# NVlabs/intrinsic3d

Measured on NVIDIA H100. Metric: gauss_newton_iterations_per_sec, higher is better.
Workload: dtype f32

## Files before the change

intrinsic3d_b200/csrc/i3d_engine.cu:

```cuda
#include <cuda_runtime.h>
#include <dlfcn.h>

#include <algorithm>
#include <chrono>
#include <climits>
#include <cmath>
#include <cstdarg>
#include <cstdio>
#include <cstdlib>
#include <cstring>
#include <string>
#include <vector>

#include "../../include/i3d_c_api.h"
#include "i3d_kernels.cuh"
#include "i3d_lighting.cuh"
#include "i3d_recolor.cuh"
#include "i3d_gridops.cuh"
#include "i3d_host.h"
#include "i3d_frames.h"
#include "i3d_fusion.h"
#include "i3d_mesh.h"
#include "i3d_render.h"
#include "i3d_track.h"
// ... 47 lines not shown
    std::string error;

    int64_t n = 0;
    float voxel_size = 0.f, truncation = 0.f;
    Dev<int32_t> x, y, z, nbr;
    Dev<double> sdf0, sdfA, albA, sdfB, albB, sh;
    Dev<float> weight;
    Dev<uchar4> rgb;
    double* sdf = nullptr; double* alb = nullptr;
    double* c_sdf = nullptr; double* c_alb = nullptr;
    bool have_sh = false;
    int F = 0, W = 0, H = 0;
    double pyr_scale = 1.0;
    Dev<float> lum, depth;
    Dev<float> tile_min, tile_max;
    Dev<unsigned long long> cull_stats;
    Dev<double> camA, camB;
    double* cam = nullptr; double* c_cam = nullptr;
    bool have_cam = false;
    Dev<uint8_t> flags;
    Dev<int32_t> up_xyz, up_vals; Dev<uint8_t> up_rgb; Dev<unsigned long long> up_keys; Dev<int> up_dup; Dev<double> up_sh;
    uint64_t hash_cap = 0;
    Dev<int32_t> sp_x, sp_y, sp_z; Dev<double> sp_sdf0, sp_sdf, sp_alb; Dev<float> sp_w; Dev<uchar4> sp_rgb;
    Dev<int32_t> act, scan_counts, scan_total;
    int n_active = 0, K = 0, stride = 0;
    Dev<float> Rt;
    Dev<FramePose> pose_ctx, pose_ctx_c;
    Dev<int32_t> obs_frame, row_frame;
    Dev<float> obs_w;
    Dev<float4> Jt;
    Dev<float2> Jtail;
    Dev<double> row_res, row_wraw;
    Dev<float> ea_w;
    Dev<double> lap;
    Dev<float> cam_acc;
    Dev<double> minv, type_w;
    Dev<int> fail_flag;
    Dev<float> v_bg, v_cg, v_s, v_jtj, v_b, v_x, v_r, v_z, v_p, v_ps, v_qg, v_tr, v_delta;
    Dev<double> v_bgd, v_cgd, v_qgd, cam_accd;
    Dev<CgCtl> ctl;
    Dev<double> red_partials, red_out;
    Dev<unsigned int> red_counters;
    size_t max_blocks = 0;
    bool keep_raw = false;
    Dev<float> dbg_v;
    I3DParams last_params{};
    bool have_iter = false;
    Timing timing;
    int64_t launches = 0;
    int64_t host_syncs = 0;
    Dev<IterDev> iter_dev;
    int last_cg_iterations = 4, prev_cg_iterations = 4;
    bool pcg_fused = true;
    int64_t step_n = -1;
    unsigned step_grid = 0; int step_K = 0; size_t step_smem = 0;
    Dev<uint8_t> color;
    bool have_color = false;
    Dev<unsigned long long> recolor_counts;
    Dev<int32_t> sv_table, sv_index, sv_nbr;
    Dev<int> sv_scalars, sv_deg;
    Dev<double> sv_acc, sv_work;
    Dev<I3DLightingInfo> sv_info;
    Dev<uint8_t> sh_has;
    int sv_S = 0;
    double* sv_x = nullptr;
    SubvolGrid sv_grid{};
    FusionState fusion;
    ScoreScratch scores;
    RgbdStore rgbd;
    SensorStore sensor;
    MeshState mesh;
    RenderState render;
    TrackScratch track;
    int64_t shard_begin = 0, shard_end = -1;
    int rank = 0, world = 1;
    NcclApi::Comm comm = nullptr;
    bool shard_ready = false;
    Dev<uint8_t> held;
    Dev<uint8_t> held_mask;
    Dev<int32_t> slist;
    int64_t n_shared = 0;
    int64_t hv0 = 0, hv1 = 0;
    int64_t loc_begin = 0, loc_end = 0;
    Dev<double> xbuf;
    Dev<uint8_t> mbox;
    size_t mbox_cap = 0;
    bool p2p_ready = false;
    unsigned int xseq = 0;
    std::vector<void*> peer_base;
    Dev<double*> d_peer_data;
    Dev<unsigned int*> d_peer_flags;
    static constexpr size_t kMboxFlagBytes = 4096;
    P2PView p2p_view() const { P2PView v; v.rank = rank; v.world = world; v.peer_data = d_peer_data.p; v.peer_flags = d_peer_flags.p; v.cap = mbox_cap; return v; }
    Shard shard() const
    {
        Shard sh;
        if (world > 1) { sh.own_begin = shard_begin; sh.own_end = shard_end; sh.hv0 = hv0; sh.hv1 = hv1; sh.cam_owner = (rank == 0); sh.defer = 1; sh.loc_begin = loc_begin; sh.loc_end = loc_end; }
        else { sh.own_begin = 0; sh.own_end = n; sh.hv0 = 0; sh.hv1 = n; sh.cam_owner = 1; sh.defer = 0; sh.loc_begin = 0; sh.loc_end = n; }
        return sh;
    }
    int64_t held_count() const { return (world > 1 ? 2 * (hv1 - hv0) : 2 * n) + 6 * static_cast<int64_t>(F) + 9; }
    ShareView share_view() const { ShareView v; v.n_shared = n_shared; v.slist = slist.p; v.held = held_mask.p; return v; }

    int64_t U() const { return 2 * n + 6 * static_cast<int64_t>(F) + 9; }
    ReduceSite site(int s)
    {
// ... 162 lines not shown
    rows.n_active = e->n_active; rows.K = e->K; rows.stride = e->stride; rows.act = e->act.p; rows.Jt = e->Jt.p; rows.Jtail = e->Jtail.p;
    rows.row_frame = e->row_frame.p; rows.row_res = e->row_res.p; rows.row_wraw = e->row_wraw.p;
    return rows;
}

RegView reg_view(I3DEngine* e, const I3DParams& P)
{
    RegView rv;
    rv.flags = e->flags.p; rv.ea_w = e->ea_w.p; rv.lap = e->lap.p;
    rv.use_er = P.use_er; rv.use_es = P.use_es; rv.use_ea = P.use_ea;
    return rv;
}

SelectCam select_cam(const I3DEngine* e, const double hc9[9], float occlusion)
{
    SelectCam sc;
    sc.fx = static_cast<float>(hc9[0] * e->pyr_scale); sc.fy = static_cast<float>(hc9[1] * e->pyr_scale);
    sc.cx = static_cast<float>(hc9[2] * e->pyr_scale); sc.cy = static_cast<float>(hc9[3] * e->pyr_scale);
    sc.dist_zero = 1;
    for (int k = 0; k < 5; ++k) { sc.d[k] = static_cast<float>(hc9[4 + k]); if (sc.d[k] != 0.0f) sc.dist_zero = 0; }
    sc.occlusion = occlusion;
    return sc;
}

CullView cull_view(const I3DEngine* e, unsigned long long* stats)
{
    static const bool no_cull = std::getenv("I3D_NO_CULL") != nullptr;
    return CullView{e->tile_min.p, e->tile_max.p, no_cull ? 0 : 1, stats};
}

#define NK(call)                                                            \
    do {                                                                    \
        int _r = (call);                                                    \
        if (_r != 0) throw NcclError{_r, __LINE__};                         \
    } while (0)


bool pdl_enabled() { static const bool on = [] { const char* v = std::getenv("I3D_PDL"); return !(v && v[0] == '0'); }(); return on; }

template <bool COOPERATIVE = false, class... KArgs, class... Args>
void pdl_launch(I3DEngine* e, void (*kern)(KArgs...), unsigned grid, unsigned block, size_t smem, Args&&... args)
{
    cudaLaunchConfig_t cfg{};
    cfg.gridDim = dim3(grid); cfg.blockDim = dim3(block); cfg.dynamicSmemBytes = smem; cfg.stream = e->stream;
    cudaLaunchAttribute at[2];
    unsigned na = 0;
    if (COOPERATIVE) { at[na].id = cudaLaunchAttributeCooperative; at[na].val.cooperative = 1; ++na; }
    if (pdl_enabled()) { at[na].id = cudaLaunchAttributeProgrammaticStreamSerialization; at[na].val.programmaticStreamSerializationAllowed = 1; ++na; }
    cfg.attrs = at; cfg.numAttrs = na;
    CK(cudaLaunchKernelEx(&cfg, kern, static_cast<KArgs>(args)...));
    e->launches += 1;
}

template <int MODE>
void launch_eg_rows(I3DEngine* e, const GridView& g, const CamView& cv, const EgRows& rows, const int32_t* obs_frame, const float* obs_w)
{
    if constexpr (MODE == ROWS_COST)
    {
        const size_t smem = rows_smem_bytes(MODE, 256, true, e->F);
        if (2 * (smem + 1024) <= 227u * 1024u)
        {
            auto kern = k_eg_rows<MODE, 256, true>;
            CK(cudaFuncSetAttribute(kern, cudaFuncAttributeMaxDynamicSharedMemorySize, static_cast<int>(smem)));
            pdl_launch(e, kern, blocks_for(static_cast<size_t>(rows.stride), 256), 256, smem, g, e->frame_view(), cv, rows, obs_frame, obs_w, e->site(SITE_EG_COST));
            return;
        }
    }
    auto kern = k_eg_rows<MODE, 128, false>;
    const size_t smem = rows_smem_bytes(MODE, 128, false, e->F);
    CK(cudaFuncSetAttribute(kern, cudaFuncAttributeMaxDynamicSharedMemorySize, static_cast<int>(smem)));
    pdl_launch(e, kern, blocks_for(static_cast<size_t>(rows.stride), 128), 128, smem, g, e->frame_view(), cv, rows, obs_frame, obs_w, e->site(SITE_EG_COST));
}

void allreduce_scalars(I3DEngine* e, double* dev, int count, int kind, int respect_done)
{
    if (e->world <= 1) return;
    if (e->p2p_ready && count <= 30)
    {
        const unsigned int seq = ++e->xseq;
        pdl_launch(e, k_xchg_scalars, 1, 32, 0, e->p2p_view(), seq, dev, count, e->ctl.p, kind, respect_done);
        return;
    }
    NK(g_nccl.AllReduce(dev, dev, static_cast<size_t>(count), NCCL_FLOAT64, NCCL_SUM, e->comm, e->stream));
    if (kind >= 0) pdl_launch(e, k_epilogue, 1, 32, 0, e->ctl.p, dev, kind, respect_done);
}

void exchange(I3DEngine* e, float* v0, float* v1, float* extra_f, int n_extra_f, double* extra_d, int n_extra_d, int respect_done, int epilogue_kind = -1)
{
    if (e->world <= 1) return;
    const ShareView shv = e->share_view();
    const size_t nv = v1 ? 2 : 1;
    const size_t total = nv * static_cast<size_t>(e->n_shared) + n_extra_f + n_extra_d;
    const size_t threads = static_cast<size_t>(e->n_shared) + n_extra_f + n_extra_d;
    if (e->p2p_ready && total <= e->mbox_cap)
    {
        const unsigned int seq = ++e->xseq;
        double* buf = reinterpret_cast<double*>(e->mbox.p + I3DEngine::kMboxFlagBytes) + static_cast<size_t>(seq & 1u) * e->mbox_cap;
        pdl_launch(e, k_pack, blocks_for(threads), kThreads, 0, shv, v0, v1, extra_f, n_extra_f, extra_d, n_extra_d, buf, e->ctl.p, respect_done);
        pdl_launch(e, k_xchg_pull, blocks_for(threads), kThreads, 0, e->p2p_view(), seq, shv, v0, v1, extra_f, n_extra_f, extra_d, n_extra_d, e->ctl.p, respect_done, epilogue_kind);
        return;
    }
    e->xbuf.ensure(2 * static_cast<size_t>(e->n_shared) + CamAccLayout{e->F}.size() + 64);
    pdl_launch(e, k_pack, blocks_for(threads), kThreads, 0, shv, v0, v1, extra_f, n_extra_f, extra_d, n_extra_d, e->xbuf.p, e->ctl.p, respect_done);
    NK(g_nccl.AllReduce(e->xbuf.p, e->xbuf.p, total, NCCL_FLOAT64, NCCL_SUM, e->comm, e->stream));
    pdl_launch(e, k_unpack, blocks_for(threads), kThreads, 0, shv, v0, v1, extra_f, n_extra_f, extra_d, n_extra_d, e->xbuf.p, e->ctl.p, respect_done);
    if (epilogue_kind >= 0) pdl_launch(e, k_epilogue, 1, 32, 0, e->ctl.p, extra_d, epilogue_kind, respect_done);
}

size_t apply_smem_bytes(int F, int K)
{
    return static_cast<size_t>((6 * F + 9 + 15) & ~15) * sizeof(double) + static_cast<size_t>(14 + 6 * K) * kThreads * sizeof(float);
}

size_t accum_smem_bytes(int F, int K)
{
    return static_cast<size_t>((CamAccLayout{F}.size() + 15) & ~15) * sizeof(double) + static_cast<size_t>(K) * 8 * kThreads * sizeof(float);
}

int check_frame_limit(I3DEngine* e, int F, int K)
{
    int optin = 0;
    CK(cudaDeviceGetAttribute(&optin, cudaDevAttrMaxSharedMemoryPerBlockOptin, e->device));
    cudaFuncAttributes fa_acc{}, fa_app{};
    CK(cudaFuncGetAttributes(&fa_acc, k_eg_accum));
// ... 425 lines not shown
    double hc9[9];
    CK(cudaMemcpyAsync(hc9, e->cam + 6 * static_cast<size_t>(F), 9 * sizeof(double), cudaMemcpyDeviceToHost, st));
    CK(cudaStreamSynchronize(st));
    const SelectCam sc = select_cam(e, hc9, 0.0f);
    if (!(std::isfinite(sc.fx) && sc.fx > 0.0f && std::isfinite(sc.fy) && sc.fy > 0.0f && std::isfinite(sc.cx) && std::isfinite(sc.cy)))
        return fail(e, "i3d_render_keyframes: the camera needs finite intrinsics with fx, fy > 0 (fx %g, fy %g, cx %g, cy %g after pyr_scale %g)",
                    sc.fx, sc.fy, sc.cx, sc.cy, e->pyr_scale);
    for (int k = 0; k < 5; ++k)
        if (!std::isfinite(sc.d[k])) return fail(e, "i3d_render_keyframes: distortion coefficient %d is not finite", k);
    RenderCam cam;
    cam.fx = sc.fx; cam.fy = sc.fy; cam.cx = sc.cx; cam.cy = sc.cy; cam.dist_zero = sc.dist_zero;
    for (int k = 0; k < 5; ++k) cam.d[k] = sc.d[k];
    e->render.rt.ensure(12 * static_cast<size_t>(F));
    k_pose_mats<<<blocks_for(F, 64), 64, 0, st>>>(F, e->cam, e->render.rt.p);
    render::keyframes(e->render, e->timing, render_grid(e, P.sdf_source, P.photometric != 0), cam, e->render.rt.p, n, ids, e->W, e->H, e->depth.p,
                      e->lum.p, P.planes, P.photometric != 0, stats, st);
    return 0;
}

}

extern "C" {

int i3d_abi_version(void) { return I3D_ABI_VERSION; }
uint64_t i3d_sizeof_params(void) { return sizeof(I3DParams); }
uint64_t i3d_sizeof_iter_info(void) { return sizeof(I3DIterInfo); }

void i3d_default_params(I3DParams* p)
{
    std::memset(p, 0, sizeof(*p));
    p->lambda[0] = 0.2; p->lambda[1] = 80.0; p->lambda[2] = 120.0; p->lambda[3] = 0.1;
    p->use_er = p->use_es = p->use_ea = 1;
    p->occlusion_distance = 0.02f; p->num_observations = 5; p->lm_steps = 50;
    p->initial_trust_region_radius = 1e4; p->max_trust_region_radius = 1e16; p->min_trust_region_radius = 1e-32;
    p->min_relative_decrease = 1e-3; p->min_lm_diagonal = 1e-6; p->max_lm_diagonal = 1e32; p->eta = 0.1;
    p->function_tolerance = 1e-6; p->gradient_tolerance = 1e-10; p->parameter_tolerance = 1e-8;
    p->max_linear_solver_iterations = 500; p->min_linear_solver_iterations = 0; p->residual_reset_period = 10;
    p->max_consecutive_invalid_steps = 5;
}

int i3d_engine_create(int device, I3DEngine** out)
{
    *out = nullptr;
    int count = 0;
    cudaError_t err = cudaGetDeviceCount(&count);
    if (err != cudaSuccess || count <= 0) return fail(nullptr, "i3d_engine_create: no CUDA device available (%s); this engine has no CPU fallback", cudaGetErrorString(err));
    if (device < 0 || device >= count) return fail(nullptr, "i3d_engine_create: device %d out of range (%d devices)", device, count);
    cudaDeviceProp prop;
    if (cudaGetDeviceProperties(&prop, device) != cudaSuccess) return fail(nullptr, "i3d_engine_create: cannot query device %d", device);
    if (prop.major != 9 || prop.minor != 0) return fail(nullptr, "i3d_engine_create: device %d is sm_%d%d; this library is built for sm_90a (H100) only", device, prop.major, prop.minor);
    I3DEngine* e = new I3DEngine();
    e->device = device;
    { const char* v = std::getenv("I3D_PCG_FUSED"); e->pcg_fused = !(v && v[0] == '0'); }
    const int rc = guarded(e, [&]() {
        CK(cudaStreamCreateWithFlags(&e->stream, cudaStreamNonBlocking));
        e->timing.pool.resize(4096);
        for (auto& ev : e->timing.pool) CK(cudaEventCreate(&ev));
        return 0;
    });
    if (rc != 0) { g_create_error = e->error; delete e; return rc; }
    *out = e;
    return 0;
}

void i3d_engine_destroy(I3DEngine* e)
{
    if (!e) return;
    cudaSetDevice(e->device);
    cudaStreamSynchronize(e->stream);
    for (size_t r = 0; r < e->peer_base.size(); ++r)
        if (static_cast<int>(r) != e->rank && e->peer_base[r]) cudaIpcCloseMemHandle(e->peer_base[r]);
    if (e->comm && g_nccl.CommDestroy) g_nccl.CommDestroy(e->comm);
    for (auto& ev : e->timing.pool) cudaEventDestroy(ev);
    if (e->mesh.ev_ready) for (auto& ev : e->mesh.ev) cudaEventDestroy(ev);
    cudaStreamDestroy(e->stream);
    delete e;
}

const char* i3d_last_error(const I3DEngine* e) { return e ? e->error.c_str() : g_create_error.c_str(); }

int i3d_upload_grid(I3DEngine* e, int64_t n, const int32_t* xyz, const double* sdf0, const double* sdf_refined, const double* albedo,
                    const float* weight, const uint8_t* rgb, float voxel_size)
{
    if (!e) return 1;
    if (n <= 0 || n > (1ll << 30)) return fail(e, "i3d_upload_grid: bad voxel count %lld", static_cast<long long>(n));
    return guarded(e, [&]() {
        cudaStream_t st = e->stream;
        e->n = n; e->voxel_size = voxel_size; e->truncation = voxel_size * 5.0f;
        forget_voxel_set(e);
        e->x.ensure(n); e->y.ensure(n); e->z.ensure(n); e->nbr.ensure(static_cast<size_t>(NB_COUNT) * n);
        e->sdf0.ensure(n); e->sdfA.ensure(n); e->sdfB.ensure(n); e->albA.ensure(n); e->albB.ensure(n); e->weight.ensure(n); e->rgb.ensure(n);
        e->sdf = e->sdfA.p; e->c_sdf = e->sdfB.p; e->alb = e->albA.p; e->c_alb = e->albB.p;
        e->up_xyz.ensure(3 * static_cast<size_t>(n)); e->up_rgb.ensure(3 * static_cast<size_t>(n));
        CK(cudaMemcpyAsync(e->up_xyz.p, xyz, 3 * n * sizeof(int32_t), cudaMemcpyHostToDevice, st));
        CK(cudaMemcpyAsync(e->up_rgb.p, rgb, 3 * n, cudaMemcpyHostToDevice, st));
        CK(cudaMemcpyAsync(e->sdf0.p, sdf0, n * sizeof(double), cudaMemcpyHostToDevice, st));
        CK(cudaMemcpyAsync(e->sdf, sdf_refined, n * sizeof(double), cudaMemcpyHostToDevice, st));
        CK(cudaMemcpyAsync(e->alb, albedo, n * sizeof(double), cudaMemcpyHostToDevice, st));
        CK(cudaMemcpyAsync(e->weight.p, weight, n * sizeof(float), cudaMemcpyHostToDevice, st));
        k_deinterleave_xyz<<<blocks_for(n), kThreads, 0, st>>>(n, e->up_xyz.p, e->x.p, e->y.p, e->z.p, e->up_rgb.p, e->rgb.p);
        const int hdup = rebuild_topology(e);
        if (hdup) return fail(e, "i3d_upload_grid: duplicate voxel coordinates");
        return 0;
    });
}

// ... 1348 lines not shown
```

intrinsic3d_b200/csrc/i3d_kernels.cuh:

```cuda
#pragma once
#include <cuda_runtime.h>
#include <cooperative_groups.h>
#include <stdint.h>
#include <limits.h>
#include "i3d_math.cuh"
#include "i3d_grid.cuh"
#include "i3d_observe.cuh"
#include "../../include/i3d_types.h"

namespace i3d
{

enum : uint8_t { FL_VALID = 1, FL_ACTIVE = 2, FL_RING = 4, FL_FREE_SDF = 8, FL_FREE_ALB = 16, FL_ES_JAC = 32, FL_ROW = 64  };

struct Shard
{
    int64_t own_begin, own_end;
    int64_t hv0, hv1;
    int cam_owner;
    int defer;
    int64_t loc_begin, loc_end;
    __device__ __forceinline__ bool owns_voxel(int64_t v) const { return v >= own_begin && v < own_end; }
    __device__ __forceinline__ bool owns_unknown(int64_t j, int64_t n) const
    {
// ... 480 lines not shown
    for (int k = 0; k < 10; ++k) s10[k] = sdf[idx[k]];
#pragma unroll
    for (int k = 0; k < 4; ++k) a4[k] = alb[idx[10 + k]];
    return true;
}

__device__ __forceinline__ double sdf_to_weight(double sdf, double truncation)
{
    const double a = fmin(fabs(sdf), truncation) / truncation;
    return fmin(fmax(1.0 - a, 0.01), 1.0);
}

struct CamAccLayout
{
    int F;
    __host__ __device__ int pose_stride() const { return 33; }
    __host__ __device__ int tail() const { return 33 * F; }
    __host__ __device__ int size() const { return 33 * F + 43; }
};

enum { ROWS_BUILD = 0, ROWS_COST = 1 };
constexpr int kRowThreads = 128;

__device__ __forceinline__ uint32_t smem_u32(const void* p) { return static_cast<uint32_t>(__cvta_generic_to_shared(p)); }
__device__ __forceinline__ void mbar_init(uint64_t* bar, uint32_t count)
{
    asm volatile("mbarrier.init.shared::cta.b64 [%0], %1;" ::"r"(smem_u32(bar)), "r"(count) : "memory");
    asm volatile("fence.mbarrier_init.release.cluster;" ::: "memory");
}
__device__ __forceinline__ void mbar_expect_tx(uint64_t* bar, uint32_t bytes)
{
    asm volatile("mbarrier.arrive.expect_tx.shared::cta.b64 _, [%0], %1;" ::"r"(smem_u32(bar)), "r"(bytes) : "memory");
}
__device__ __forceinline__ void bulk_copy_g2s(void* dst_smem, const void* src_gmem, uint32_t bytes , uint64_t* bar)
{
    asm volatile("cp.async.bulk.shared::cluster.global.mbarrier::complete_tx::bytes [%0], [%1], %2, [%3];"
                 ::"r"(smem_u32(dst_smem)), "l"(src_gmem), "r"(bytes), "r"(smem_u32(bar)) : "memory");
}
__device__ __forceinline__ void mbar_wait(uint64_t* bar, uint32_t parity)
{
    uint32_t done = 0;
    while (!done)
        asm volatile("{\n\t.reg .pred P1;\n\tmbarrier.try_wait.parity.shared::cta.b64 P1, [%1], %2;\n\tselp.b32 %0, 1, 0, P1;\n\t}"
                     : "=r"(done) : "r"(smem_u32(bar)), "r"(parity) : "memory");
}

static_assert(kVoxelGeomWords == 15, "VoxelGeom size changed: update the pose-table staging boundary and its test");
__host__ __device__ inline size_t rows_pose_bytes(int F) { return (static_cast<size_t>(F) * sizeof(FramePose) + 127) & ~static_cast<size_t>(127); }
__host__ __device__ inline size_t rows_smem_bytes(int mode, int threads, bool stage, int F)
{
    return (stage ? 128 + rows_pose_bytes(F) : 0) + static_cast<size_t>(threads) * (kVoxelGeomWords * sizeof(double) + (mode == ROWS_BUILD ? kVoxelDerivWords * sizeof(float) : 0));
}

template <int MODE, int THREADS, bool STAGE>
__global__ void __launch_bounds__(THREADS, THREADS == 128 ? 4 : 2)
k_eg_rows(GridView g, FrameView fr, CamView cv, EgRows rows, const int32_t* __restrict__ obs_frame, const float* __restrict__ obs_w, ReduceSite site)
{
    extern __shared__ __align__(128) unsigned char s_rows[];
    pdl_prologue();
    uint64_t* s_bar = reinterpret_cast<uint64_t*>(s_rows);
    const FramePose* s_pose = reinterpret_cast<const FramePose*>(s_rows + 128);
    unsigned char* s_state = s_rows + (STAGE ? 128 + rows_pose_bytes(fr.F) : 0);
    double* s_vg = reinterpret_cast<double*>(s_state);
    float* s_vd = reinterpret_cast<float*>(s_state + static_cast<size_t>(THREADS) * kVoxelGeomWords * sizeof(double));
    if (STAGE)
    {
        if (threadIdx.x == 0)
        {
            const uint32_t bytes = static_cast<uint32_t>(fr.F * sizeof(FramePose));
            mbar_init(s_bar, 1);
            mbar_expect_tx(s_bar, bytes);
            bulk_copy_g2s(s_rows + 128, cv.fpose, bytes, s_bar);
        }
        __syncthreads();
    }
    const int a = blockIdx.x * blockDim.x + threadIdx.x;
    double acc[1] = {0.0};
    const VoxelGeomView vg{s_vg + threadIdx.x, THREADS};
    const VoxelDerivView vd{s_vd + threadIdx.x, THREADS};
    bool ok = a < rows.n_active;
    double wsdf = 0.0;
    if (ok)
    {
        const int64_t v = rows.act[a];
        int32_t idx[14];
        double s10[10], a4[4];
        ok = gather_stencil(g, g.sdf, g.albedo, v, idx, s10, a4);
        if (ok)
        {
            double sh[9];
#pragma unroll
            for (int k = 0; k < 9; ++k) sh[k] = g.sh[static_cast<int64_t>(k) * g.n + v];
            const int coord[3] = {g.x[v], g.y[v], g.z[v]};
            VoxelGeom vg_r;
            VoxelDeriv vd_r;
            voxel_geom_make<MODE == ROWS_BUILD>(s10, a4, coord, static_cast<double>(g.voxel_size), sh, &vg_r, &vd_r);
            voxel_geom_park(vg_r, s_vg + threadIdx.x, THREADS);
            if (MODE == ROWS_BUILD) voxel_deriv_park(vd_r, s_vd + threadIdx.x, THREADS);
            if (MODE == ROWS_BUILD) wsdf = sdf_to_weight(s10[0], static_cast<double>(g.truncation));
        }
    }
    if (STAGE) mbar_wait(s_bar, 0);
    if (a < rows.stride)
    {
        CamParams<double> cam;
        make_cam_params(cv, fr.pyr_scale, fr.W, fr.H, &cam);
        const size_t img_stride = static_cast<size_t>(fr.W) * fr.H;
        const int32_t* __restrict__ fsrc = (MODE == ROWS_BUILD) ? obs_frame : rows.row_frame;
        int f_next = ok ? fsrc[a] : -1;
#pragma unroll 1
        for (int k = 0; k < rows.K; ++k)
        {
            const size_t slot = static_cast<size_t>(k) * rows.stride + a;
            const int f = f_next;
            if (ok && k + 1 < rows.K) f_next = fsrc[slot + rows.stride];
            if (!STAGE && f_next >= 0)
            {
                const char* pf = reinterpret_cast<const char*>(cv.fpose + f_next);
                asm volatile("prefetch.global.L1 [%0];" ::"l"(pf));
                asm volatile("prefetch.global.L1 [%0];" ::"l"(pf + 128));
            }
            int32_t rf = -1; double res = 0.0, wraw = 0.0;
            if (f >= 0)
            {
                const FramePose& fp = STAGE ? s_pose[f] : cv.fpose[f];
                PointSave sv[4];
                float e[4];
                res = eg_frame_primal<MODE == ROWS_BUILD>(vg, fp, cam, LinearImage{fr.lum + img_stride * f}, sv, e);
                if (MODE == ROWS_BUILD)
                {
                    if (res != 0.0)
                    {
                        CamParams<float> cf;
                        cf.fx = static_cast<float>(cam.fx); cf.fy = static_cast<float>(cam.fy); cf.cx = static_cast<float>(cam.cx); cf.cy = static_cast<float>(cam.cy);
                        cf.k1 = static_cast<float>(cam.k1); cf.k2 = static_cast<float>(cam.k2); cf.k3 = static_cast<float>(cam.k3);
                        cf.p1 = static_cast<float>(cam.p1); cf.p2 = static_cast<float>(cam.p2);
                        cf.pyr_scale = static_cast<float>(cam.pyr_scale); cf.w = cam.w; cf.h = cam.h;
                        float row[29];
                        eg_frame_deriv(vd, fp, cf, sv, e, row);
                        rf = f;
                        wraw = static_cast<double>(obs_w[slot]) * wsdf;
                        rows.store_row(slot, row);
                    }
                }
                else acc[0] += rows.row_wraw[slot] * res * res;
            }
            if (MODE == ROWS_BUILD) { rows.row_frame[slot] = rf; rows.row_res[slot] = res; rows.row_wraw[slot] = wraw; }
        }
    }
    if (MODE == ROWS_COST) grid_reduce<1>(acc, site);
}

__global__ void __launch_bounds__(kThreads)
k_eg_accum(GridView g, EgRows rows, int F, double* __restrict__ bg, double* __restrict__ cg, double* __restrict__ cam_acc ,
           ReduceSite site )
{
    pdl_prologue();
    extern __shared__ double s_dyn_d[];
    const CamAccLayout lay{F};
    double* s_cam = s_dyn_d;
    float* s_park = reinterpret_cast<float*>(s_dyn_d + ((lay.size() + 15) & ~15));
    for (int i = threadIdx.x; i < lay.size(); i += blockDim.x) s_cam[i] = 0.0;
    __syncthreads();
    const int tid = threadIdx.x, lane = tid & 31;
    const int a = blockIdx.x * blockDim.x + tid;
    const bool in_range = a < rows.n_active;
    double acc[3] = {0.0, 0.0, 0.0};
    float gsum[14], csum[14];
#pragma unroll
    for (int m = 0; m < 14; ++m) { gsum[m] = 0.0f; csum[m] = 0.0f; }
    float tl[64];
#pragma unroll
    for (int i = 0; i < 64; ++i) tl[i] = 0.0f;
    int fk[I3D_MAX_OBS];
#pragma unroll
    for (int k = 0; k < I3D_MAX_OBS; ++k)
    {
        fk[k] = -1;
        if (k >= rows.K) continue;
        const size_t slot = static_cast<size_t>(k) * rows.stride + (in_range ? a : 0);
        const int f = in_range ? rows.row_frame[slot] : -1;
        fk[k] = f;
        if (f >= 0)
        {
            float row[29];
            rows.load_row<false>(slot, row);
            const double wraw = rows.row_wraw[slot], res = rows.row_res[slot];
            const float wf = static_cast<float>(wraw), wr = static_cast<float>(wraw * res);
            acc[0] += wraw; acc[1] += wraw * res * res; acc[2] += 1.0;
#pragma unroll
            for (int m = 0; m < 14; ++m) { gsum[m] += wr * row[m]; csum[m] += wf * row[m] * row[m]; }
#pragma unroll
            for (int m = 0; m < 9; ++m) { tl[m] += wr * row[20 + m]; tl[9 + m] += wf * row[20 + m] * row[20 + m]; }
            int t = 18;
#pragma unroll
            for (int r = 0; r < 4; ++r)
#pragma unroll
                for (int c = r; c < 4; ++c) tl[t++] += wf * row[20 + r] * row[20 + c];
#pragma unroll
            for (int r = 0; r < 5; ++r)
// ... 1507 lines not shown
```

intrinsic3d_b200/csrc/i3d_math.cuh:

```cuda
#pragma once

#ifndef I3D_HD
#ifdef __CUDACC__
#define I3D_HD __host__ __device__ __forceinline__
#else
#define I3D_HD inline
#endif
#endif

#include <math.h>

namespace i3d
{

#define I3D_QUAD(i, j) (((i) == 0) ? (((j) == 0) ? 0 : ((j) == 1) ? 6 : ((j) == 2) ? 1 : 4) \
                      : ((i) == 1) ? (((j) == 0) ? 6 : ((j) == 1) ? 9 : ((j) == 2) ? 7 : 8) \
                      : ((i) == 2) ? (((j) == 0) ? 1 : ((j) == 1) ? 7 : ((j) == 2) ? 2 : 3) \
                                   : (((j) == 0) ? 4 : ((j) == 1) ? 8 : ((j) == 2) ? 3 : 5))

template <class T> struct Num;
template <> struct Num<double>
{
    static I3D_HD double sqrt_(double x) { return sqrt(x); }
    static I3D_HD double floor_(double x) { return floor(x); }
// ... 591 lines not shown


template <bool GRAD>
I3D_HD double bicubic_eval(const BicubicSite& s, const float p[16], float* Lu, float* Lv)
{
    double wu[4], wv[4], du[4], dv[4];
    cr_weights<double>(s.xu, wu);
    cr_weights<double>(s.xv, wv);
    if (GRAD) { cr_dweights<double>(s.xu, du); cr_dweights<double>(s.xv, dv); }
    double L = 0.0, lu = 0.0, lv = 0.0;
#pragma unroll
    for (int i = 0; i < 4; ++i)
    {
        const double p0 = static_cast<double>(p[4 * i]), p1 = static_cast<double>(p[4 * i + 1]), p2 = static_cast<double>(p[4 * i + 2]), p3 = static_cast<double>(p[4 * i + 3]);
        const double ri = fma(wu[0], p0, fma(wu[1], p1, fma(wu[2], p2, wu[3] * p3)));
        L = fma(wv[i], ri, L);
        if (GRAD)
        {
            const double rd = fma(du[0], p0, fma(du[1], p1, fma(du[2], p2, du[3] * p3)));
            lu = fma(wv[i], rd, lu);
            lv = fma(dv[i], ri, lv);
        }
    }
    if (GRAD) { *Lu = static_cast<float>(lu); *Lv = static_cast<float>(lv); }
    return L;
}

struct PointSave { float x, y, iz, Lu, Lv; };

template <bool DERIV, class VG, class IMG>
I3D_HD double eg_frame_primal(const VG& vg, const FramePose& fp, const CamParams<double>& cam, const IMG& img,
                              PointSave sv[4], float e[4])
{
    double u[4], v[4];
    bool inb = true;
#pragma unroll
    for (int i = 0; i < 4; ++i)
    {
        const double X0 = vg.Xv(i, 0), X1 = vg.Xv(i, 1), X2 = vg.Xv(i, 2);
        const double Y0 = fp.R[0] * X0 + fp.R[1] * X1 + fp.R[2] * X2 + fp.t[0];
        const double Y1 = fp.R[3] * X0 + fp.R[4] * X1 + fp.R[5] * X2 + fp.t[1];
        const double Y2 = fp.R[6] * X0 + fp.R[7] * X1 + fp.R[8] * X2 + fp.t[2];
        const double iz = rcp_f64(Y2);
        const double x = Y0 * iz, y = Y1 * iz;
        const double r2 = x * x + y * y, r4 = r2 * r2, r6 = r4 * r2;
        const double dc = 1.0 + cam.k1 * r2 + cam.k2 * r4 + cam.k3 * r6;
        const double xd = x * dc + 2.0 * cam.p1 * x * y + cam.p2 * (r2 + 2.0 * x * x);
        const double yd = y * dc + 2.0 * cam.p2 * xd * y + cam.p1 * (r2 + 2.0 * y * y);
        u[i] = cam.fx * xd + cam.cx; v[i] = cam.fy * yd + cam.cy;
        if (u[i] < 0.0 || u[i] > static_cast<double>(cam.w - 1) || v[i] < 0.0 || v[i] > static_cast<double>(cam.h - 1)) inb = false;
        if (DERIV) { sv[i].x = static_cast<float>(x); sv[i].y = static_cast<float>(y); sv[i].iz = static_cast<float>(iz); }
    }
    double L[4];
#pragma unroll
    for (int i = 0; i < 4; i += 2)
    {
        BicubicSite s0, s1;
        bicubic_locate(u[i], v[i], cam.w, cam.h, &s0);
        bicubic_locate(u[i + 1], v[i + 1], cam.w, cam.h, &s1);
        float p0[16], p1[16];
        img.taps2(cam.w, cam.h, s0, s1, p0, p1);
        float lu = 0.0f, lv = 0.0f;
        L[i] = bicubic_eval<DERIV>(s0, p0, &lu, &lv);
        if (DERIV) { sv[i].Lu = lu; sv[i].Lv = lv; }
        L[i + 1] = bicubic_eval<DERIV>(s1, p1, &lu, &lv);
        if (DERIV) { sv[i + 1].Lu = lu; sv[i + 1].Lv = lv; }
    }
    if (!inb) return 0.0;
    const double d1 = vg.dSv(0) - (L[1] - L[0]);
    const double d2 = vg.dSv(1) - (L[2] - L[0]);
    const double d3 = vg.dSv(2) - (L[3] - L[0]);
    const double r = sqrt(d1 * d1 + d2 * d2 + d3 * d3);
    if (!finite_(r)) return 0.0;
    if (DERIV && r != 0.0)
    {
        const double ir = 1.0 / r;
        e[0] = static_cast<float>(-(d1 + d2 + d3) * ir); e[1] = static_cast<float>(d1 * ir); e[2] = static_cast<float>(d2 * ir); e[3] = static_cast<float>(d3 * ir);
    }
    return r;
}

template <class VD>
I3D_HD void eg_frame_deriv(const VD& vd, const FramePose& fp, const CamParams<float>& cam, const PointSave sv[4], const float e[4],
                           float* __restrict__ row)
{
#pragma unroll
    for (int k = 0; k < 29; ++k) row[k] = 0.0f;
    float m[3] = {0.0f, 0.0f, 0.0f};
    float tacc[3] = {0.0f, 0.0f, 0.0f};
#define I3D_POINT_DERIV(POINT)                                                                                                        \
    {                                                                                                                                 \
        const int i = POINT;                                                                                                          \
        const float x = sv[i].x, y = sv[i].y, iz = sv[i].iz, Lu = sv[i].Lu, Lv = sv[i].Lv, ei = e[i];                                 \
        const float r2 = x * x + y * y, r4 = r2 * r2, r6 = r4 * r2;                                                                   \
        const float dc = 1.0f + cam.k1 * r2 + cam.k2 * r4 + cam.k3 * r6;                                                              \
        const float dcp = cam.k1 + 2.0f * cam.k2 * r2 + 3.0f * cam.k3 * r4;                                                           \
        const float xd = x * dc + 2.0f * cam.p1 * x * y + cam.p2 * (r2 + 2.0f * x * x);                                               \
        const float yd = y * dc + 2.0f * cam.p2 * xd * y + cam.p1 * (r2 + 2.0f * y * y);                                              \
        const float xdx = dc + 2.0f * x * x * dcp + 2.0f * cam.p1 * y + 6.0f * cam.p2 * x;                                            \
        const float xdy = 2.0f * x * y * dcp + 2.0f * cam.p1 * x + 2.0f * cam.p2 * y;                                                 \
        const float ydx = 2.0f * x * y * dcp + 2.0f * cam.p2 * y * xdx + 2.0f * cam.p1 * x;                                           \
        const float ydy = dc + 2.0f * y * y * dcp + 2.0f * cam.p2 * (y * xdy + xd) + 6.0f * cam.p1 * y;                              \
        const float gu = Lu * cam.fx, gv = Lv * cam.fy;                                                                               \
        const float Lx = gu * xdx + gv * ydx, Ly = gu * xdy + gv * ydy;                                                               \
        const float LY0 = Lx * iz, LY1 = Ly * iz, LY2 = -(Lx * x + Ly * y) * iz;                                                      \
        const float LX0 = LY0 * fp.Rf[0] + LY1 * fp.Rf[3] + LY2 * fp.Rf[6];                                                           \
        const float LX1 = LY0 * fp.Rf[1] + LY1 * fp.Rf[4] + LY2 * fp.Rf[7];                                                           \
        const float LX2 = LY0 * fp.Rf[2] + LY1 * fp.Rf[5] + LY2 * fp.Rf[8];                                                           \
        const float s = vd.sv(i), g0 = vd.gv(i, 0), g1 = vd.gv(i, 1), g2 = vd.gv(i, 2);                                              \
        const float Xf0 = vd.X0v(0) + (i == 1 ? vd.hv() : 0.0f) - g0 * s;                                                            \
        const float Xf1 = vd.X0v(1) + (i == 2 ? vd.hv() : 0.0f) - g1 * s;                                                            \
        const float Xf2 = vd.X0v(2) + (i == 3 ? vd.hv() : 0.0f) - g2 * s;                                                            \
        const float c0 = fp.small ? LY0 : LX0, c1 = fp.small ? LY1 : LX1, c2 = fp.small ? LY2 : LX2;                                  \
        m[0] += ei * (Xf1 * c2 - Xf2 * c1); m[1] += ei * (Xf2 * c0 - Xf0 * c2); m[2] += ei * (Xf0 * c1 - Xf1 * c0);                   \
        tacc[0] += ei * LY0; tacc[1] += ei * LY1; tacc[2] += ei * LY2;                                                                \
        row[20] -= ei * (Lu * cam.pyr_scale * xd);                                                                                    \
        row[21] -= ei * (Lv * cam.pyr_scale * yd);                                                                                    \
        row[22] -= ei * (Lu * cam.pyr_scale);                                                                                         \
// ... 36 lines not shown
```

Baseline: 141.2.

## Add optional warp-compacted row evaluation and hoist bicubic site location

Adds a COMPACT variant of the edge-gradient rows kernel. Each warp ballots which (observation, voxel) slots are valid and redistributes the valid work densely across lanes, so lanes with no observation do not sit idle. In cost mode the partial results are shuffled back to the owning lane before the weighted accumulation. The variant only runs when I3D_ROWS_COMPACT=1. Separately, bicubic_locate is computed for all four points before the tap loads, which is always active and may let the loads be issued earlier at the cost of more live registers.

```diff
diff --git a/intrinsic3d_b200/csrc/i3d_engine.cu b/intrinsic3d_b200/csrc/i3d_engine.cu
--- a/intrinsic3d_b200/csrc/i3d_engine.cu
+++ b/intrinsic3d_b200/csrc/i3d_engine.cu
@@ -123,6 +123,7 @@
     Dev<IterDev> iter_dev;
     int last_cg_iterations = 4, prev_cg_iterations = 4;
     bool pcg_fused = true;
+    bool rows_compact = false;
     int64_t step_n = -1;
     unsigned step_grid = 0; int step_K = 0; size_t step_smem = 0;
     Dev<uint8_t> color;
@@ -391,24 +392,30 @@
     e->launches += 1;
 }
 
-template <int MODE>
-void launch_eg_rows(I3DEngine* e, const GridView& g, const CamView& cv, const EgRows& rows, const int32_t* obs_frame, const float* obs_w)
+template <int MODE, bool COMPACT>
+void launch_eg_rows_as(I3DEngine* e, const GridView& g, const CamView& cv, const EgRows& rows, const int32_t* obs_frame, const float* obs_w)
 {
     if constexpr (MODE == ROWS_COST)
     {
         const size_t smem = rows_smem_bytes(MODE, 256, true, e->F);
         if (2 * (smem + 1024) <= 227u * 1024u)
         {
-            auto kern = k_eg_rows<MODE, 256, true>;
+            auto kern = k_eg_rows<MODE, 256, true, COMPACT>;
             CK(cudaFuncSetAttribute(kern, cudaFuncAttributeMaxDynamicSharedMemorySize, static_cast<int>(smem)));
             pdl_launch(e, kern, blocks_for(static_cast<size_t>(rows.stride), 256), 256, smem, g, e->frame_view(), cv, rows, obs_frame, obs_w, e->site(SITE_EG_COST));
             return;
         }
     }
-    auto kern = k_eg_rows<MODE, 128, false>;
+    auto kern = k_eg_rows<MODE, 128, false, COMPACT>;
     const size_t smem = rows_smem_bytes(MODE, 128, false, e->F);
     CK(cudaFuncSetAttribute(kern, cudaFuncAttributeMaxDynamicSharedMemorySize, static_cast<int>(smem)));
     pdl_launch(e, kern, blocks_for(static_cast<size_t>(rows.stride), 128), 128, smem, g, e->frame_view(), cv, rows, obs_frame, obs_w, e->site(SITE_EG_COST));
+}
+template <int MODE>
+void launch_eg_rows(I3DEngine* e, const GridView& g, const CamView& cv, const EgRows& rows, const int32_t* obs_frame, const float* obs_w)
+{
+    if (e->rows_compact) launch_eg_rows_as<MODE, true>(e, g, cv, rows, obs_frame, obs_w);
+    else launch_eg_rows_as<MODE, false>(e, g, cv, rows, obs_frame, obs_w);
 }
 
 void allreduce_scalars(I3DEngine* e, double* dev, int count, int kind, int respect_done)
@@ -940,6 +947,7 @@
     I3DEngine* e = new I3DEngine();
     e->device = device;
     { const char* v = std::getenv("I3D_PCG_FUSED"); e->pcg_fused = !(v && v[0] == '0'); }
+    { const char* v = std::getenv("I3D_ROWS_COMPACT"); e->rows_compact = v && v[0] == '1'; }
     const int rc = guarded(e, [&]() {
         CK(cudaStreamCreateWithFlags(&e->stream, cudaStreamNonBlocking));
         e->timing.pool.resize(4096);
diff --git a/intrinsic3d_b200/csrc/i3d_kernels.cuh b/intrinsic3d_b200/csrc/i3d_kernels.cuh
--- a/intrinsic3d_b200/csrc/i3d_kernels.cuh
+++ b/intrinsic3d_b200/csrc/i3d_kernels.cuh
@@ -556,7 +556,19 @@
     return (stage ? 128 + rows_pose_bytes(F) : 0) + static_cast<size_t>(threads) * (kVoxelGeomWords * sizeof(double) + (mode == ROWS_BUILD ? kVoxelDerivWords * sizeof(float) : 0));
 }
 
-template <int MODE, int THREADS, bool STAGE>
+__device__ __forceinline__ int nth_set_bit(uint32_t m, int n)
+{
+    int pos = 0;
+#pragma unroll
+    for (int w = 16; w > 0; w >>= 1)
+    {
+        const int c = __popc(m & ((1u << w) - 1u));
+        if (n >= c) { n -= c; m >>= w; pos += w; }
+    }
+    return pos;
+}
+
+template <int MODE, int THREADS, bool STAGE, bool COMPACT>
 __global__ void __launch_bounds__(THREADS, THREADS == 128 ? 4 : 2)
 k_eg_rows(GridView g, FrameView fr, CamView cv, EgRows rows, const int32_t* __restrict__ obs_frame, const float* __restrict__ obs_w, ReduceSite site)
 {
@@ -580,8 +592,6 @@
     }
     const int a = blockIdx.x * blockDim.x + threadIdx.x;
     double acc[1] = {0.0};
-    const VoxelGeomView vg{s_vg + threadIdx.x, THREADS};
-    const VoxelDerivView vd{s_vd + threadIdx.x, THREADS};
     bool ok = a < rows.n_active;
     double wsdf = 0.0;
     if (ok)
@@ -605,51 +615,139 @@
         }
     }
     if (STAGE) mbar_wait(s_bar, 0);
-    if (a < rows.stride)
-    {
-        CamParams<double> cam;
-        make_cam_params(cv, fr.pyr_scale, fr.W, fr.H, &cam);
-        const size_t img_stride = static_cast<size_t>(fr.W) * fr.H;
-        const int32_t* __restrict__ fsrc = (MODE == ROWS_BUILD) ? obs_frame : rows.row_frame;
-        int f_next = ok ? fsrc[a] : -1;
+    CamParams<double> cam;
+    make_cam_params(cv, fr.pyr_scale, fr.W, fr.H, &cam);
+    const size_t img_stride = static_cast<size_t>(fr.W) * fr.H;
+    const int32_t* __restrict__ fsrc = (MODE == ROWS_BUILD) ? obs_frame : rows.row_frame;
+    auto row_eval = [&](int col, size_t slot, int f, double wsdf_v, int32_t& rf, double& wraw) -> double {
+        const VoxelGeomView vg{s_vg + col, THREADS};
+        const VoxelDerivView vd{s_vd + col, THREADS};
+        const FramePose& fp = STAGE ? s_pose[f] : cv.fpose[f];
+        PointSave sv[4];
+        float e[4];
+        const double res = eg_frame_primal<MODE == ROWS_BUILD>(vg, fp, cam, LinearImage{fr.lum + img_stride * f}, sv, e);
+        if (MODE == ROWS_BUILD)
+        {
+            if (res != 0.0)
+            {
+                CamParams<float> cf;
+                cf.fx = static_cast<float>(cam.fx); cf.fy = static_cast<float>(cam.fy); cf.cx = static_cast<float>(cam.cx); cf.cy = static_cast<float>(cam.cy);
+                cf.k1 = static_cast<float>(cam.k1); cf.k2 = static_cast<float>(cam.k2); cf.k3 = static_cast<float>(cam.k3);
+                cf.p1 = static_cast<float>(cam.p1); cf.p2 = static_cast<float>(cam.p2);
+                cf.pyr_scale = static_cast<float>(cam.pyr_scale); cf.w = cam.w; cf.h = cam.h;
+                float row[29];
+                eg_frame_deriv(vd, fp, cf, sv, e, row);
+                rf = f;
+                wraw = static_cast<double>(obs_w[slot]) * wsdf_v;
+                rows.store_row(slot, row);
+            }
+        }
+        return res;
+    };
+    if (!COMPACT)
+    {
+        if (a < rows.stride)
+        {
+            int f_next = ok ? fsrc[a] : -1;
 #pragma unroll 1
-        for (int k = 0; k < rows.K; ++k)
-        {
-            const size_t slot = static_cast<size_t>(k) * rows.stride + a;
-            const int f = f_next;
-            if (ok && k + 1 < rows.K) f_next = fsrc[slot + rows.stride];
-            if (!STAGE && f_next >= 0)
+            for (int k = 0; k < rows.K; ++k)
+            {
+                const size_t slot = static_cast<size_t>(k) * rows.stride + a;
+                const int f = f_next;
+                if (ok && k + 1 < rows.K) f_next = fsrc[slot + rows.stride];
+                if (!STAGE && f_next >= 0)
+                {
+                    const char* pf = reinterpret_cast<const char*>(cv.fpose + f_next);
+                    asm volatile("prefetch.global.L1 [%0];" ::"l"(pf));
+                    asm volatile("prefetch.global.L1 [%0];" ::"l"(pf + 128));
+                }
+                int32_t rf = -1; double res = 0.0, wraw = 0.0;
+                if (f >= 0)
+                {
+                    res = row_eval(threadIdx.x, slot, f, wsdf, rf, wraw);
+                    if (MODE == ROWS_COST) acc[0] += rows.row_wraw[slot] * res * res;
+                }
+                if (MODE == ROWS_BUILD) { rows.row_frame[slot] = rf; rows.row_res[slot] = res; rows.row_wraw[slot] = wraw; }
+            }
+        }
+    }
+    else
+    {
+        constexpr uint32_t FULL = 0xffffffffu;
+        const int lane = threadIdx.x & 31;
+        const int a0 = a - lane;
+        const int c0 = threadIdx.x - lane;
+        __syncwarp();
+        uint32_t bal[I3D_MAX_OBS];
+#pragma unroll
+        for (int k = 0; k < I3D_MAX_OBS; ++k) bal[k] = __ballot_sync(FULL, ok && k < rows.K && fsrc[static_cast<size_t>(k) * rows.stride + a] >= 0);
+        if (MODE == ROWS_BUILD && a < rows.stride)
+        {
+#pragma unroll
+            for (int k = 0; k < I3D_MAX_OBS; ++k)
+                if (k < rows.K && !((bal[k] >> lane) & 1u))
+                {
+                    const size_t slot = static_cast<size_t>(k) * rows.stride + a;
+                    rows.row_frame[slot] = -1; rows.row_res[slot] = 0.0; rows.row_wraw[slot] = 0.0;
+                }
+        }
+        int total = 0;
+#pragma unroll
+        for (int k = 0; k < I3D_MAX_OBS; ++k) total += __popc(bal[k]);
+        auto locate = [&](int q, int& kq, int& tq) {
+            int base = 0, n = 0;
+            uint32_t m = 0;
+            kq = -1;
+#pragma unroll
+            for (int k = 0; k < I3D_MAX_OBS; ++k)
+            {
+                const int c = __popc(bal[k]);
+                if (q >= base && q < base + c) { kq = k; m = bal[k]; n = q - base; }
+                base += c;
+            }
+            tq = kq >= 0 ? nth_set_bit(m, n) : lane;
+        };
+        int kn, tn;
+        locate(lane, kn, tn);
+        int f_next = kn >= 0 ? fsrc[static_cast<size_t>(kn) * rows.stride + a0 + tn] : -1;
+#pragma unroll 1
+        for (int q0 = 0; q0 < total; q0 += 32)
+        {
+            const int k = kn, t = tn, f = f_next;
+            const size_t slot = static_cast<size_t>(k < 0 ? 0 : k) * rows.stride + a0 + t;
+            locate(q0 + 32 + lane, kn, tn);
+            if (kn >= 0) f_next = fsrc[static_cast<size_t>(kn) * rows.stride + a0 + tn];
+            if (!STAGE && kn >= 0)
             {
                 const char* pf = reinterpret_cast<const char*>(cv.fpose + f_next);
                 asm volatile("prefetch.global.L1 [%0];" ::"l"(pf));
                 asm volatile("prefetch.global.L1 [%0];" ::"l"(pf + 128));
             }
-            int32_t rf = -1; double res = 0.0, wraw = 0.0;
-            if (f >= 0)
-            {
-                const FramePose& fp = STAGE ? s_pose[f] : cv.fpose[f];
-                PointSave sv[4];
-                float e[4];
-                res = eg_frame_primal<MODE == ROWS_BUILD>(vg, fp, cam, LinearImage{fr.lum + img_stride * f}, sv, e);
-                if (MODE == ROWS_BUILD)
+            const double wsdf_t = (MODE == ROWS_BUILD) ? __shfl_sync(FULL, wsdf, t) : 0.0;
+            double res = 0.0;
+            if (k >= 0)
+            {
+                int32_t rf = -1; double wraw = 0.0;
+                res = row_eval(c0 + t, slot, f, wsdf_t, rf, wraw);
+                if (MODE == ROWS_BUILD) { rows.row_frame[slot] = rf; rows.row_res[slot] = res; rows.row_wraw[slot] = wraw; }
+            }
+            if (MODE == ROWS_COST)
+            {
+                int base = 0;
+#pragma unroll
+                for (int kk = 0; kk < I3D_MAX_OBS; ++kk)
                 {
-                    if (res != 0.0)
+                    const int c = __popc(bal[kk]);
+                    if (base < q0 + 32 && base + c > q0)
                     {
-                        CamParams<float> cf;
-                        cf.fx = static_cast<float>(cam.fx); cf.fy = static_cast<float>(cam.fy); cf.cx = static_cast<float>(cam.cx); cf.cy = static_cast<float>(cam.cy);
-                        cf.k1 = static_cast<float>(cam.k1); cf.k2 = static_cast<float>(cam.k2); cf.k3 = static_cast<float>(cam.k3);
-                        cf.p1 = static_cast<float>(cam.p1); cf.p2 = static_cast<float>(cam.p2);
-                        cf.pyr_scale = static_cast<float>(cam.pyr_scale); cf.w = cam.w; cf.h = cam.h;
-                        float row[29];
-                        eg_frame_deriv(vd, fp, cf, sv, e, row);
-                        rf = f;
-                        wraw = static_cast<double>(obs_w[slot]) * wsdf;
-                        rows.store_row(slot, row);
+                        const int p = base + __popc(bal[kk] & ((1u << lane) - 1u)) - q0;
+                        const bool mine = ((bal[kk] >> lane) & 1u) && p >= 0 && p < 32;
+                        const double r = __shfl_sync(FULL, res, mine ? p : lane);
+                        if (mine) acc[0] += rows.row_wraw[static_cast<size_t>(kk) * rows.stride + a] * r * r;
                     }
+                    base += c;
                 }
-                else acc[0] += rows.row_wraw[slot] * res * res;
-            }
-            if (MODE == ROWS_BUILD) { rows.row_frame[slot] = rf; rows.row_res[slot] = res; rows.row_wraw[slot] = wraw; }
+            }
         }
     }
     if (MODE == ROWS_COST) grid_reduce<1>(acc, site);
diff --git a/intrinsic3d_b200/csrc/i3d_math.cuh b/intrinsic3d_b200/csrc/i3d_math.cuh
--- a/intrinsic3d_b200/csrc/i3d_math.cuh
+++ b/intrinsic3d_b200/csrc/i3d_math.cuh
@@ -667,18 +667,18 @@
         if (DERIV) { sv[i].x = static_cast<float>(x); sv[i].y = static_cast<float>(y); sv[i].iz = static_cast<float>(iz); }
     }
     double L[4];
+    BicubicSite st[4];
+#pragma unroll
+    for (int i = 0; i < 4; ++i) bicubic_locate(u[i], v[i], cam.w, cam.h, &st[i]);
 #pragma unroll
     for (int i = 0; i < 4; i += 2)
     {
-        BicubicSite s0, s1;
-        bicubic_locate(u[i], v[i], cam.w, cam.h, &s0);
-        bicubic_locate(u[i + 1], v[i + 1], cam.w, cam.h, &s1);
         float p0[16], p1[16];
-        img.taps2(cam.w, cam.h, s0, s1, p0, p1);
+        img.taps2(cam.w, cam.h, st[i], st[i + 1], p0, p1);
         float lu = 0.0f, lv = 0.0f;
-        L[i] = bicubic_eval<DERIV>(s0, p0, &lu, &lv);
+        L[i] = bicubic_eval<DERIV>(st[i], p0, &lu, &lv);
         if (DERIV) { sv[i].Lu = lu; sv[i].Lv = lv; }
-        L[i + 1] = bicubic_eval<DERIV>(s1, p1, &lu, &lv);
+        L[i + 1] = bicubic_eval<DERIV>(st[i + 1], p1, &lu, &lv);
         if (DERIV) { sv[i + 1].Lu = lu; sv[i + 1].Lv = lv; }
     }
     if (!inb) return 0.0;
```

Result: no change. 141.7 (median of 6 runs) (+0.4%).
